# chenruduan/OAReactDiff

Measured on AMD Instinct MI355X. Metric: denoising_steps_per_sec, higher is better.
Workload: dtype f32; 1 GPU; EGNNDynamics.forward (LEFTNet H=196 R=96 L=6), B=64 reactions/GPU x 3 objects x 23 atoms, complete graph per reaction (N=4416, E=300288), T=1000 sampler step shape; batch_per_gpu=64, atoms_per_object=23, parallelism=replica x1 (no collective), launch=eager

## Files before the change

### oareactdiff_amd/_capi.py

```python
from __future__ import annotations

import ctypes as C
import os

from .build import LIB

OARD_MAX_OBJECTS = 8
ABI_VERSION = 2040
OARD_OK, OARD_EINVAL, OARD_ENOTCOMPLETE, OARD_EHIP, OARD_ENOMEM = 0, -1, -2, -3, -4
ERRORS = {OARD_EINVAL: "invalid argument / unsupported configuration", OARD_ENOTCOMPLETE: "topology is not complete-per-sample",
          OARD_EHIP: "HIP runtime error", OARD_ENOMEM: "workspace too small"}

PREC_GCL_BF16X3, PREC_EQUI_BF16X3, PREC_TRAIN_BF16X3 = 1, 2, 4
TAP_S, TAP_VEC, TAP_EDGE, TAP_POS_FRAME, TAP_DPOS, TAP_HOUT, TAP_LABELS, TAP_NE1 = 1, 2, 3, 4, 5, 6, 7, 8

EXPORTS = ["oard_version", "oard_supported", "oard_param_count", "oard_packed_bytes", "oard_pack_weights",
           "oard_topology_create", "oard_topology_destroy", "oard_topology_num_nodes", "oard_topology_num_edges",
           "oard_topology_num_inner_edges", "oard_topology_num_samples", "oard_topology_check_edge_index",
           "oard_workspace_bytes", "oard_forward", "oard_active_inner_edges", "oard_debug_lin3u_table", "oard_sampler_step", "oard_sampler_step_dev", "oard_tap", "oard_debug_stop_after", "oard_debug_option", "oard_timing_enable", "oard_timing_reset",
           "oard_timing_get",
           "oard_topology_create_parts", "oard_topology_export", "oard_tape_bytes", "oard_tape_entry", "oard_forward_train",
           "oard_packed_bwd_bytes", "oard_pack_weights_bwd", "oard_gcl_backward_dx", "oard_edge_node_sums",
           "oard_equi_backward_dx", "oard_scalarize_backward", "oard_equi_msg_backward", "oard_lin3u_forward", "oard_lin3u_backward", "oard_wgrad_scratch_bytes", "oard_wgrad",
           "oard_train_scratch_bytes", "oard_train_scratch_poison", "oard_train_scratch_entry", "oard_train_tail_backward",
# ... 99 lines not shown
    L.oard_train_stage_backward.restype = ci
    L.oard_nan_replace.argtypes = [cfgp, vp, vp, pvp, pvp, vp]; L.oard_nan_replace.restype = ci
    pf, cf = C.POINTER(C.c_float), C.c_float
    L.oard_loss_prepare.argtypes = [cfgp, vp, pvp, pvp, pvp, pvp, vp, vp, ci, pf, pf, ci, ci, pvp, pvp, vp]; L.oard_loss_prepare.restype = ci
    L.oard_loss_terms.argtypes = [cfgp, vp, pvp, pvp, pvp, pvp, pvp, vp, vp, ci, pf, pf, pf, ci, ci, vp, vp, pvp, vp]; L.oard_loss_terms.restype = ci
    cd = C.c_double
    L.oard_adamw_step.argtypes = [vp, vp, vp, vp, vp, i64, cd, cd, cd, cd, cd, i64, ci, cd, vp]; L.oard_adamw_step.restype = ci
    L.oard_adamw_step_dev.argtypes = [vp, vp, vp, vp, vp, i64, cd, cd, cd, cd, cd, ci, ci, vp, ci, vp, vp, vp, vp]; L.oard_adamw_step_dev.restype = ci
    L.oard_library_stream.argtypes = [ci, pvp]; L.oard_library_stream.restype = ci
    L.oard_graph_create.argtypes = [cfgp, vp, vp, i64, vp, i64, pvp]; L.oard_graph_create.restype = ci
    L.oard_graph_destroy.argtypes = [vp]; L.oard_graph_destroy.restype = None
    L.oard_graph_num_nodes.argtypes = [vp]; L.oard_graph_num_nodes.restype = i64
    L.oard_graph_num_edges.argtypes = [vp]; L.oard_graph_num_edges.restype = i64
    L.oard_graph_object_rows.argtypes = [vp, ci]; L.oard_graph_object_rows.restype = i64
    L.oard_graph_is_complete.argtypes = [vp]; L.oard_graph_is_complete.restype = ci
    L.oard_graph_workspace_bytes.argtypes = [cfgp, vp]; L.oard_graph_workspace_bytes.restype = sz
    L.oard_graph_forward.argtypes = [cfgp, vp, pvp, sz, pvp, vp, ci, vp, pvp, vp, sz, vp, vp]; L.oard_graph_forward.restype = ci
    L.oard_debug_stop_after.argtypes = [C.c_int]; L.oard_debug_stop_after.restype = C.c_int
    L.oard_debug_option.argtypes = [C.c_char_p, C.c_int]; L.oard_debug_option.restype = C.c_int
    L.oard_timing_enable.argtypes = [C.c_int]; L.oard_timing_enable.restype = C.c_int
    L.oard_timing_reset.argtypes = []; L.oard_timing_reset.restype = C.c_int
    L.oard_timing_get.argtypes = [C.c_char_p, C.POINTER(C.c_double), C.POINTER(i64)]; L.oard_timing_get.restype = C.c_int
    for env, opt in (("OARD_GCL_VARIANT", b"gcl_variant"), ("OARD_EQUI_VARIANT", b"equi_variant"),
                     ("OARD_NODE_VARIANT", b"node_variant"), ("OARD_GCL_SKIP", b"gcl_skip"), ("OARD_EQUI_SKIP", b"equi_skip"), ("OARD_GCL_PERSIST", b"gcl_persist"), ("OARD_GCL_GRID", b"gcl_grid"), ("OARD_PARTS", b"parts"), ("OARD_SEQUENTIAL", b"sequential"), ("OARD_POISON", b"poison"), ("OARD_AUTO_SMALL", b"auto_small"), ("OARD_AUTO_TINY", b"auto_tiny"), ("OARD_NPB", b"npb"),
                     ("OARD_WGRAD_WGS", b"wgrad_wgs"), ("OARD_WGRAD_LDS", b"wgrad_lds"), ("OARD_WGRAD_T16", b"wgrad_t16"), ("OARD_WGRAD_QUEUE", b"wgrad_queue"), ("OARD_GATE_FOLD", b"gate_fold"), ("OARD_WGRAD_SHAPES", b"wgrad_shapes"), ("OARD_TRAIN_DUAL", b"train_dual"), ("OARD_SMALL_SPLIT", b"small_split"),
                     ("OARD_SKIP_FAMILIES", b"skip_families")):
        if os.environ.get(env) not in (None, ""):
            check(L.oard_debug_option(opt, int(os.environ[env])), f"oard_debug_option({opt.decode()})")
    _lib = L
    return L


def timing_get(family: str):
    ms, n = C.c_double(0.0), C.c_int64(0)
    check(lib().oard_timing_get(family.encode(), C.byref(ms), C.byref(n)), "oard_timing_get")
    return ms.value, n.value
```

### oareactdiff_amd/csrc/oard_edge_v1.h

```cpp
#pragma once
#include "oard_kernels.h"

typedef __attribute__((address_space(3))) void* lds_ptr_t;
typedef const __attribute__((address_space(1))) void* gbl_ptr_t;

OARD_DEV void glds16(const float* gsrc_lane, float* lds_chunk);
OARD_DEV void glds16u(const float* chunk_uniform, unsigned lane_byte_off, float* lds_chunk) {
    glds16(reinterpret_cast<const float*>(reinterpret_cast<const char*>(chunk_uniform) + lane_byte_off), lds_chunk);
}
OARD_DEV void glds16(const float* gsrc_lane, float* lds_chunk) {
#ifndef OARD_ABL_NODMA_INSTR
    __builtin_amdgcn_global_load_lds((gbl_ptr_t)gsrc_lane, (lds_ptr_t)lds_chunk, 16, 0, 0);
#else
    asm volatile("" :: "v"(gsrc_lane), "s"(lds_chunk));
#endif
}

OARD_DEV void phase_barrier() {
    asm volatile("s_waitcnt vmcnt(0)" ::: "memory");
#ifndef OARD_ABL_NOBARRIER
    __syncthreads();
#endif
}

// ... 427 lines not shown
            if (TRAIN) st_f4(tape.z3 + e * D::WP + 4 * g + 16 * t, pendz[gg]);
        }
    }
    PROBE_END(pf);
    TL_END();
}

template <class D>
struct EquiStream {
    static constexpr int WB = D::WB, D1T = D::D1T, RB = D::RB, HT = D::HT;
    static constexpr int G1 = D1T, G2 = 1 + D1T + RB, NG2 = 3 * HT;
    static constexpr bool ROWS4 = (D::H % 16) >= 1 && (D::H % 16) <= 4;
    static constexpr int SLAB = G2 > G1 ? G2 : G1;
    static constexpr int NPH = WB + NG2;
    static constexpr int C1 = WB * G1, CHUNKS = C1 + NG2 * G2;
    static constexpr size_t LDS_BYTES = (size_t)2 * SLAB * 1024;
};

template <class D, int WAVES, bool TRAIN>
__global__ __launch_bounds__(WAVES * 64) void k_equi_edge_v1(TopoDev tp, const float* __restrict__ stream,
                                                             const float* __restrict__ dp0b,
                                                             const float* __restrict__ ew, const float* __restrict__ rbuf,
                                                             float* __restrict__ qbuf, float* __restrict__ zd1,
                                                             float* __restrict__ cdbuf, ActList al) {
    extern __shared__ __attribute__((aligned(16))) float smem[];
    using S = EquiStream<D>;
    constexpr int WB = D::WB, D1T = D::D1T, RB = D::RB, HT = D::HT, G1 = S::G1, G2 = S::G2;
    const int lane = threadIdx.x & 63, g = lane >> 4;
    const int wave = __builtin_amdgcn_readfirstlane(threadIdx.x >> 6);

    SlabPrefetch<WAVES, S::SLAB, 0, 3> pf;
    pf.wave = wave;
    pf.lane_off = (unsigned)lane * 16u;
    auto pf_begin = [&](int p) {
        const int start = p < WB ? p * G1 : S::C1 + (p - WB) * G2;
        pf.begin(stream, smem, p, start, p >= S::NPH ? 0 : (p < WB ? G1 : G2));
    };
    auto hook = [&]() { pf.tick(); };
    auto A = [&](int p, int j) -> f4 {
        return *reinterpret_cast<const f4*>(smem + ((size_t)(p & 1) * S::SLAB + j) * 256 + lane * 4);
    };
    auto SL = [&](int p) -> const float* { return smem + (size_t)(p & 1) * S::SLAB * 256 + lane * 4; };

    const long long n_cols = al.n != nullptr ? (long long)*al.n : tp.A;
    if ((long long)blockIdx.x * WAVES * 16 >= n_cols) return;
    const long long c = ((long long)blockIdx.x * WAVES + wave) * 16 + (lane & 15);
    const bool live = c < n_cols;
    const size_t a = (size_t)(live ? (al.rows != nullptr ? (long long)al.rows[c] : c) : tp.A);
    const float* erow = ew + (live ? a : (size_t)tp.E) * D::WP + 4 * g;
    f4 d1[D1T];
#pragma unroll
    for (int t = 0; t < D1T; ++t) d1[t] = ld_vec(dp0b, t, lane);
    f4 rb[RB];
#pragma unroll
    for (int b = 0; b < RB; ++b) rb[b] = ld_blk(rbuf, a, D::RP, b, lane);
    f4 xn = ld_f4(erow);
    pf_begin(0);
    pf.flush();

    int p = 0;
    for (int b = 0; b < WB; ++b, ++p) {
        phase_barrier();
        const f4 x = xn;
        pf_begin(p + 1);
        if (b + 1 < WB) xn = ld_f4(erow + 16 * (b + 1));
        chain_kouter<D1T>(SL(p), 0, x, d1, hook);
        pf.flush();
    }
    if (TRAIN) {
#pragma unroll
        for (int t = 0; t < D1T; ++t) st_blk(zd1, a, D::D1P, t, lane, d1[t]);
    }
#pragma unroll
    for (int t = 0; t < D1T; ++t) d1[t] = silu4(d1[t]);

    float* qrow = qbuf + a * (size_t)(3 * D::HP) + 4 * g;
    float* cdrow = TRAIN ? cdbuf + a * (size_t)(3 * D::HP) + 4 * g : nullptr;
    f4 pend = f4zero(), pendc = f4zero();
    int pend_off = 0;
    auto t2_phase = [&](int i, auto rows4) {
        phase_barrier();
        if (i > 0) {
            st_f4(qrow + pend_off, pend);
            if (TRAIN) st_f4(cdrow + pend_off, pendc);
        }
        pf_begin(p + 1);
        const int tt = i / 3, th = i - 3 * tt;
        f4 cd, cr;
        if (decltype(rows4)::value) {
            cd = reduce_g(chain_tile4<D1T>(SL(p), 1, d1, A(p, 0), hook));
            cr = reduce_g(chain_tile4<RB>(SL(p), 1 + D1T, rb, f4zero(), hook));
            if (g != 0) { cd = f4zero(); cr = f4zero(); }
        } else {
            cd = chain_tile<D1T>(SL(p), 1, d1, A(p, 0), hook);
            cr = chain_tile<RB>(SL(p), 1 + D1T, rb, f4zero(), hook);
        }
        pf.flush();
        pend = cd * cr;
        if (TRAIN) pendc = cd;
        pend_off = th * D::HP + 16 * tt;
        ++p;
    };
    constexpr int N_FULL = S::ROWS4 ? S::NG2 - 3 : S::NG2;
    for (int i = 0; i < N_FULL; ++i) t2_phase(i, std::false_type{});
    for (int i = N_FULL; i < S::NG2; ++i) t2_phase(i, std::true_type{});
    st_f4(qrow + pend_off, pend);
    if (TRAIN) st_f4(cdrow + pend_off, pendc);
}

template <class D>
__global__ __launch_bounds__(256) void k_equi_agg_v1(TopoDev tp, const float* __restrict__ wb, LayerOff lo,
                                                     const float* __restrict__ qbuf, const float* __restrict__ xq,
                                                     const float* __restrict__ geo, const float* __restrict__ x1,
                                                     float* __restrict__ s, const float* __restrict__ vec_in,
                                                     float* __restrict__ vec_out, float* __restrict__ v2buf,
                                                     float* __restrict__ scal, float* __restrict__ vdot) {
    bool live; const ColId id = col_id(tp.N, live);
    if (!live) return;
    const int n = id.col, a0 = tp.act_ptr[n], cnt = tp.act_ptr[n + 1] - a0;
    const int mx = wave_max(cnt);
    const float inv_sqrt2 = 0.70710678118654752f, inv_sqrt3 = 0.57735026918962576f,
                inv_sqrt_h = 1.0f / sqrtf((float)D::H);
    f4 vx[3][D::HT], dx[D::HT];
#pragma unroll
    for (int t = 0; t < D::HT; ++t) { dx[t] = f4zero(); vx[0][t] = f4zero(); vx[1][t] = f4zero(); vx[2][t] = f4zero(); }
    for (int k = 0; k < mx; ++k)
        if (k < cnt) {
            const size_t a = (size_t)a0 + k;
// ... 63 lines not shown
```

### oareactdiff_amd/csrc/oard_hip.hip

```cpp
#include <algorithm>
#include <cmath>
#include <cstdio>
#include <cstring>
#include <map>
#include <string>
#include <vector>
#include <mutex>
#include <chrono>
#include <utility>

#include "oard_kernels.h"
#include "oard_edge_v1.h"
#include "oard_edge_p.h"
#include "oard_wgrad_t16.h"
#include "oard_edge_b3.h"
#ifdef OARD_EXPERIMENTS
#include "oard_edge_fp.h"
#endif
#include "oard_node_v1.h"
#include "oard_edge_small.h"
#include "oard_edge_bwd.h"
#include "oard_node_bwd.h"
#include "oard_rows.h"
#include "oard_inst.h"
// ... 22 lines not shown
    hipEvent_t get() {
        if (!pool.empty()) { hipEvent_t e = pool.back(); pool.pop_back(); return e; }
        hipEvent_t e; (void)hipEventCreate(&e); return e;
    }
    void flush() {
        for (auto& r : recs) {
            (void)hipEventSynchronize(r.b);
            float ms = 0.f;
            (void)hipEventElapsedTime(&ms, r.a, r.b);
            total_ms[r.fam] += ms; launches[r.fam] += 1;
            pool.push_back(r.a); pool.push_back(r.b);
        }
        recs.clear();
    }
} g_timing;
int g_stop_after = 0;
int g_gcl_variant = 2;
int g_equi_variant = 2;
int g_sequential = 0;
int g_auto_tiny = 8;
int g_auto_small = 4;
int g_npb = 0;
int g_poison = 0;
int g_parts = 0;
int g_small_split = 128;
int g_wgrad_shapes = 3;
int g_wgrad_t16 = 256;
int g_wgrad_lds = 256;
int g_wgrad_wgs = 512;
int g_gcl_persist = 1;
int g_gcl_grid = 0;
int g_equi_skip = 1;
int g_gcl_skip = 1;
int g_node_variant = 1;
int g_skip_families = 0;

struct ScopedLaunch {
    hipStream_t st; hipEvent_t a; int fam; bool on;
    ScopedLaunch(int f, hipStream_t s) : st(s), fam(f), on(g_timing.on) {
        if (on) { a = g_timing.get(); (void)hipEventRecord(a, st); }
    }
    ~ScopedLaunch() {
        if (on) { hipEvent_t b = g_timing.get(); (void)hipEventRecord(b, st); g_timing.recs.push_back({a, b, fam}); }
    }
};
#define LAUNCH(fam, kern, grid, block, stream, ...) do { ScopedLaunch sl_(fam, stream); if (!((g_skip_families >> (fam)) & 1)) \
// ... 315 lines not shown
        case 10: { LAUNCH_LDS(F_GCL_EDGE, (k_gcl_edge_v1<D, 12, 1, S1, S3, false, 3>), cdiv(r1 - r0, 16 * 12), 12 * 64,
                              (GclStream<D, 1>::LDS_BYTES), st, tp, stream, P, Q, u0, c0, r0, r1, ew_in, ew_out, mbuf, GclTape{}); return OARD_OK; }
        case 11: { LAUNCH_LDS(F_GCL_EDGE, (k_gcl_edge_v1<D, 12, 2, S1, S3, false, 3>), cdiv(r1 - r0, 16 * 12), 12 * 64,
                              (GclStream<D, 2>::LDS_BYTES), st, tp, stream, P, Q, u0, c0, r0, r1, ew_in, ew_out, mbuf, GclTape{}); return OARD_OK; }
        case 12: { LAUNCH_LDS(F_GCL_EDGE, (k_gcl_edge_v1<D, 4, 1, S1, S3, false, 3>), cdiv(r1 - r0, 16 * 4), 4 * 64,
                              (GclStream<D, 1>::LDS_BYTES), st, tp, stream, P, Q, u0, c0, r0, r1, ew_in, ew_out, mbuf, GclTape{}); return OARD_OK; }
#endif
        default: return OARD_EINVAL;
    }
}
template <class D>
int launch_gcl_v1(int prec, int variant, int conc, const TopoDev& tp, const float* wb, const LayerOff& lo, const float* stream, const float* P, const float* Q, const float* u0,
                  const float* c0, bool first, bool last, const float* ew_in, float* ew_out, float* mbuf, const GclTape* tape, hipStream_t st) {
    const long long A = tp.A, E = tp.E;
    int rc;
    const bool skip = g_gcl_skip || tape;
    if (!skip || (!first && !last)) return launch_gcl_v1s<D, true, true>(prec, variant, conc, tp, wb, lo, stream, P, Q, u0, c0, 0, E, ew_in, ew_out, mbuf, tape, st);
    rc = launch_gcl_v1s<D, true, true>(prec, variant, conc, tp, wb, lo, stream, P, Q, u0, c0, 0, A, ew_in, ew_out, mbuf, tape, st);
    if (rc != OARD_OK) return rc;
    if (first && last) return launch_gcl_v1s<D, false, false>(prec, variant, conc, tp, wb, lo, stream, P, Q, u0, c0, A, E, ew_in, ew_out, mbuf, tape, st);
    if (first) return launch_gcl_v1s<D, false, true>(prec, variant, conc, tp, wb, lo, stream, P, Q, u0, c0, A, E, ew_in, ew_out, mbuf, tape, st);
    return launch_gcl_v1s<D, true, false>(prec, variant, conc, tp, wb, lo, stream, P, Q, u0, c0, A, E, ew_in, ew_out, mbuf, tape, st);
}
#define EQUI_CASE(id, WV_) case id: { \
        LAUNCH_LDS(F_EQUI_EDGE, (k_equi_edge_v1<D, WV_, false>), cdiv(tp.A, 16 * WV_), WV_ * 64, (EquiStream<D>::LDS_BYTES), st, \
                   tp, stream, dp0b, ew, rbuf, qbuf, nullptr, nullptr, al); return OARD_OK; }
template <class D>
int launch_equi_v1(int prec, int variant, int conc, const TopoDev& tp, const float* wb, const LayerOff& lo, const float* stream, const float* dp0b, const float* ew,
                   const float* rbuf, float* qbuf, float* zd1, float* cd, hipStream_t st, float* d1s = nullptr, ActList al = ActList{}) {
    if (zd1 && (prec & OARD_PREC_TRAIN_BF16X3) && d1s) {
        LAUNCH_LDS(F_EQUI_EDGE, (k_equi_edge_b3<D, true>), cdiv(tp.A, 16 * 8), 8 * 64, (EquiB3Stream<D>::LDS_BYTES), st, tp, wb + lo.equi_b3,
                   dp0b, wb + lo.dp2b, ew, rbuf, qbuf, d1s, zd1, cd, ActList{});
        return OARD_OK;
    }
    if (zd1) {
        LAUNCH_LDS(F_EQUI_EDGE, (k_equi_edge_v1<D, 8, true>), cdiv(tp.A, 16 * 8), 8 * 64, (EquiStream<D>::LDS_BYTES), st,
                   tp, stream, dp0b, ew, rbuf, qbuf, zd1, cd, ActList{});
        return OARD_OK;
    }
    if (variant == 2 && cdiv(tp.A, 16) * conc <= 512LL * g_auto_small) variant = 1;
    if ((variant == 2 || variant == 1) && cdiv(tp.A, 16) * conc <= 512LL * g_auto_tiny) variant = 4;
    if (variant == 4) {
        if (t_small.a && cdiv(tp.A, 16) * conc <= g_small_split) {
            const long long tiles = cdiv(tp.A, 16);
            LAUNCH_LDS(F_EQUI_EDGE, (k_equi_small_s1<D, 8>), tiles * cdiv(D::D1T, 8), 512, (size_t)D::WB * 1024, st,
                       tp, wb, lo, ew, t_small.a);
            LAUNCH_LDS(F_EQUI_EDGE, (k_equi_small_s2<D, 8>), tiles * cdiv(3 * D::HT, 8), 512, (size_t)(D::D1T + D::RB) * 1024, st,
                       tp, wb, lo, (const float*)t_small.a, rbuf, qbuf);
            return OARD_OK;
        }
        LAUNCH_LDS(F_EQUI_EDGE, (k_equi_edge_small<D, 8>), cdiv(tp.A, 16), 512, (EquiSmall<D>::LDS_BYTES), st,
                   tp, wb, lo, ew, rbuf, qbuf);
        return OARD_OK;
    }
    if (variant == 2 && (prec & OARD_PREC_EQUI_BF16X3) && d1s) {
        LAUNCH_LDS(F_EQUI_EDGE, (k_equi_edge_b3<D>), cdiv(tp.A, 16 * 8), 8 * 64, (EquiB3Stream<D>::LDS_BYTES), st, tp, wb + lo.equi_b3,
                   dp0b, wb + lo.dp2b, ew, rbuf, qbuf, d1s, nullptr, nullptr, al);
        return OARD_OK;
    }
    switch (variant) {
        EQUI_CASE(1, 4)
        EQUI_CASE(2, 8)
        default: return OARD_EINVAL;
    }
}

struct TapeOff {
    size_t hin, geo, rbuf, pp0, x1;
    size_t s_in[OARD_MAX_LAYERS + 1], vec_in[OARD_MAX_LAYERS + 1];
    size_t agg[OARD_MAX_LAYERS], s_mid[OARD_MAX_LAYERS];
    size_t s_a[OARD_MAX_LAYERS], vec_a[OARD_MAX_LAYERS];
    size_t ew[OARD_MAX_LAYERS + 1];
    size_t z1[OARD_MAX_LAYERS], z2[OARD_MAX_LAYERS], att[OARD_MAX_LAYERS], z3[OARD_MAX_LAYERS];
    size_t zd1[OARD_MAX_LAYERS], cd[OARD_MAX_LAYERS];
    size_t total;
};
static TapeOff make_tape(const oard_config* c, const TopoDev& td) {
    const RDims d(c->hidden, c->num_radial);
    const size_t N = td.N, E = td.E + 1, A = td.A + 1;
    TapeOff t;
    memset(&t, 0, sizeof(t));
    size_t cur = 0;
    auto take = [&](size_t bytes) { size_t o = cur; cur = align_up(cur + bytes, 256); return o; };
    t.hin = take(N * 16 * 4); t.geo = take(A * GEO_STRIDE * 4); t.rbuf = take(A * d.RP * 4); t.pp0 = take(N * 4); t.x1 = take(N * 3 * 4);
    for (int l = 0; l <= c->num_layers; ++l) {
// ... 101 lines not shown
                GclTape gt{};
                if (train) gt = GclTape{(float*)(tape + to.z1[l]), (float*)(tape + to.z2[l]), (float*)(tape + to.att[l]), (float*)(tape + to.z3[l])};
                int rc = launch_gcl_v1<D>(c->precision, gcl_variant, topo->conc, tp, wb, lo, wb + lo.gcl_stream, P, Q, wb + po.u0, wb + po.c0row, l == 0,
                                          l == c->num_layers - 1, ew_in, ew_out, mbuf, train ? &gt : nullptr, st);
                if (rc != OARD_OK) return rc;
            }
        }
        const bool rows = tp.npb <= 4;
        if (nv1 && rows) LAUNCH(F_NODE, (k_gcl_node_v1<D, NW, true>), gN16, NW * 64, st, tp, wb, lo, (const float*)xhb, (const float*)mbuf, s_mid_at(l), xq,
                                train ? (float*)(tape + to.agg[l]) : nullptr);
        else if (nv1) LAUNCH(F_NODE, (k_gcl_node_v1<D, NW, false>), gN16, NW * 64, st, tp, wb, lo, (const float*)xhb, (const float*)mbuf, s_mid_at(l), xq,
                             train ? (float*)(tape + to.agg[l]) : nullptr);
        else if constexpr (kV0) LAUNCH(F_NODE, (k_gcl_node<D>), gN, 256, st, tp, wb, lo, (const float*)xhb, (const float*)mbuf, s, xq);
        else return OARD_EINVAL;
        if (stop_after == 100 + 10 * l + 1) { topo->vec_final = (size_t)((char*)vcur - ws); return OARD_OK; }
        if (equi_variant == 0) {
            if constexpr (kV0) {
                if (A > 0) LAUNCH(F_EQUI_EDGE, (k_equi_edge<D>), gA, 256, st, tp, wb, lo, (const float*)ew_out, (const float*)rbuf,
                                  (const float*)geo, (const float*)xq, (const float*)vcur, xmsg, vmsg);
                LAUNCH(F_NODE, (k_equi_agg<D>), gN, 256, st, tp, wb, lo, (const float*)xmsg, (const float*)vmsg, (const float*)x1,
                       s, vcur, v2buf, scal, vdot);
            } else return OARD_EINVAL;
        } else {
            if (A > 0) {
                int rc = launch_equi_v1<D>(c->precision, equi_variant, topo->conc, tp, wb, lo, wb + lo.equi_stream, wb + lo.dp0b, ew_out, rbuf, vmsg,
                                           train ? (float*)(tape + to.zd1[l]) : nullptr, train ? (float*)(tape + to.cd[l]) : nullptr, st,
                                           (float*)(ws + w.d1s), al);
                if (rc != OARD_OK) return rc;
            }
#define EQUI_NODE_V1(ROWS_, XC_) LAUNCH(F_NODE, (k_equi_node_v1<D, NW, ROWS_, XC_>), gN16, NW * 64, st, tp, wb, lo, (const float*)vmsg, \
                       (const float*)xq, (const float*)geo, (const float*)x1, (const float*)s_mid_at(l), s_at(l + 1), (const float*)vcur, vnext, \
                       train ? (float*)(tape + to.s_a[l]) : nullptr, train ? (float*)(tape + to.vec_a[l]) : nullptr, al)
            if (nv1 && rows) {
                if (lo.xcross) EQUI_NODE_V1(true, true); else EQUI_NODE_V1(true, false);
            } else if (nv1) {
                if (lo.xcross) EQUI_NODE_V1(false, true); else EQUI_NODE_V1(false, false);
            } else if constexpr (kV0) {
                LAUNCH(F_NODE, (k_equi_agg_v1<D>), gN, 256, st, tp, wb, lo, (const float*)vmsg, (const float*)xq,
                       (const float*)geo, (const float*)x1, s, (const float*)vcur, vnext, v2buf, scal, vdot);
            } else return OARD_EINVAL;
            std::swap(vcur, vnext);
        }
        if constexpr (kV0) {
            if (!nv1) LAUNCH(F_NODE, (k_equi_upd<D>), gN, 256, st, tp, wb, lo, (const float*)scal, (const float*)vdot,
                             (const float*)v2buf, s, vcur);
        }
        if (stop_after == 100 + 10 * l + 2) { topo->vec_final = (size_t)((char*)vcur - ws); return OARD_OK; }
    }
    if (!train) topo->vec_final = (size_t)((char*)vcur - ws);
    if (train) {
        ZeroRows z;
        z.count = 0;
        auto add = [&](size_t off, size_t row, int ld) {
            if (z.count == 64) { LAUNCH(F_OTHER, k_zero_rows, 64, 256, st, z); z.count = 0; }
            z.p[z.count] = (float*)(tape + off) + row * (size_t)ld; z.n[z.count] = ld; ++z.count;
        };
        for (int l = 0; l <= c->num_layers; ++l) {
            add(to.ew[l], (size_t)E, D::WP);
            if (l == c->num_layers) break;
// ... 1478 lines not shown
            case OARD_TAP_EDGE:
                if (tp.E > 0)
                    hipLaunchKernelGGL(k_tap_edges, dim3((unsigned)cdiv(tp.E * d.W, 256)), dim3(256), 0, st, tp,
                                       (const float*)(ws + w.ew), d.WP, d.W, dst);
                break;
            default: return OARD_EINVAL;
        }
    }
    HIP_TRY(hipGetLastError());
    return OARD_OK;
}

int oard_debug_stop_after(int code) { g_stop_after = code; return OARD_OK; }
int oard_debug_option(const char* name, int value) {
    if (!name) return OARD_EINVAL;
    if (!kV0 && value == 0 && (strcmp(name, "gcl_variant") == 0 || strcmp(name, "equi_variant") == 0 || strcmp(name, "node_variant") == 0))
        return OARD_EINVAL;
    if (strcmp(name, "gcl_variant") == 0) { g_gcl_variant = value; return OARD_OK; }
    if (strcmp(name, "equi_variant") == 0) { g_equi_variant = value; return OARD_OK; }
    if (strcmp(name, "node_variant") == 0) { g_node_variant = value; return OARD_OK; }
    if (strcmp(name, "experiments") == 0) return kV0 ? OARD_OK : OARD_EINVAL;
    if (strcmp(name, "gcl_skip") == 0) { g_gcl_skip = value; return OARD_OK; }
    if (strcmp(name, "equi_skip") == 0) { g_equi_skip = value; return OARD_OK; }
    if (strcmp(name, "gcl_persist") == 0) { g_gcl_persist = value; return OARD_OK; }
    if (strcmp(name, "gcl_grid") == 0) { g_gcl_grid = value; return OARD_OK; }
    if (strcmp(name, "skip_families") == 0) { g_skip_families = value; return OARD_OK; }
    if (strcmp(name, "parts") == 0) { g_parts = value; return OARD_OK; }
    if (strcmp(name, "sequential") == 0) { g_sequential = value; return OARD_OK; }
    if (strcmp(name, "poison") == 0) { g_poison = value; return OARD_OK; }
    if (strcmp(name, "auto_small") == 0) { g_auto_small = value; return OARD_OK; }
    if (strcmp(name, "auto_tiny") == 0) { g_auto_tiny = value; return OARD_OK; }
    if (strcmp(name, "npb") == 0) { g_npb = value; return OARD_OK; }
    if (strcmp(name, "wgrad_wgs") == 0) { g_wgrad_wgs = value; return OARD_OK; }
    if (strcmp(name, "wgrad_t16") == 0) { g_wgrad_t16 = value; return OARD_OK; }
    if (strcmp(name, "wgrad_queue") == 0) { g_wgrad_queue = value; return OARD_OK; }
    if (strcmp(name, "gate_fold") == 0) { g_gate_fold = value; return OARD_OK; }
    if (strcmp(name, "wgrad_lds") == 0) { g_wgrad_lds = value; return OARD_OK; }
    if (strcmp(name, "wgrad_shapes") == 0) { g_wgrad_shapes = value & 3; return OARD_OK; }
    if (strcmp(name, "train_dual") == 0) { g_train_dual = value; return OARD_OK; }
    if (strcmp(name, "small_split") == 0) { g_small_split = value; return OARD_OK; }
    return OARD_EINVAL;
}
#ifdef OARD_PHASE_PROBE
int oard_debug_probe_read(unsigned long long* out8) {
    if (!out8) return OARD_EINVAL;
    HIP_TRY(hipDeviceSynchronize());
// ... 38 lines not shown
```

### oareactdiff_amd/csrc/oard_inst.h

```cpp
#pragma once
#if !defined(OARD_EXPERIMENTS) && !defined(OARD_SINGLE_TU)

#define OARD_UNPAREN(...) __VA_ARGS__
#ifdef OARD_INST_DEFINE
#define OARD_INST(K, ARGS) template __global__ void OARD_UNPAREN K ARGS;
#else
#define OARD_INST(K, ARGS) extern template __global__ void OARD_UNPAREN K ARGS;
#endif
#ifndef OARD_DIMS_LIST
#define OARD_DIMS_LIST X(196, 96) X(32, 8) X(32, 32)
#endif
#define OARD_BOOL4(M, D) M(D, true, true) M(D, false, true) M(D, true, false) M(D, false, false)

#define OARD_NW(h) (((h) + 15) / 16 <= 16 ? ((h) + 15) / 16 : 8)
#define OARD_A_GCL (TopoDev, const float*, const float*, const float*, const float*, const float*, long long, long long, const float*, float*, float*, GclTape)

#if !defined(OARD_INST_DEFINE) || defined(OARD_INST_UNIT_GCL_P)
#define OARD_I_GCL_P(D, S1, S3) OARD_INST((k_gcl_edge_p<OARD_UNPAREN D, S1, S3, false>), OARD_A_GCL) OARD_INST((k_gcl_edge_p<OARD_UNPAREN D, S1, S3, true>), OARD_A_GCL)
#define X(h, r) OARD_BOOL4(OARD_I_GCL_P, (Dims<h, r>))
OARD_DIMS_LIST
#undef X
#endif

#if !defined(OARD_INST_DEFINE) || defined(OARD_INST_UNIT_GCL_V1)
#define OARD_I_GCL_V1(D, S1, S3) \
    OARD_INST((k_gcl_edge_v1<OARD_UNPAREN D, 8, 2, S1, S3, false, 2, 3>), OARD_A_GCL) OARD_INST((k_gcl_edge_v1<OARD_UNPAREN D, 8, 2, S1, S3, true, 2, 3>), OARD_A_GCL) \
    OARD_INST((k_gcl_edge_v1<OARD_UNPAREN D, 4, 2, S1, S3, false, 2, 2>), OARD_A_GCL) \
    OARD_INST((k_gcl_edge_small<OARD_UNPAREN D, 8, S1, S3>), (TopoDev, const float*, LayerOff, const float*, const float*, const float*, const float*, long long, long long, float*, float*))
#define X(h, r) OARD_BOOL4(OARD_I_GCL_V1, (Dims<h, r>))
OARD_DIMS_LIST
#undef X
#endif

#if !defined(OARD_INST_DEFINE) || defined(OARD_INST_UNIT_B3)
#define OARD_A_EQUI_B3 (TopoDev, const float*, const float*, const float*, const float*, const float*, float*, float*, float*, float*, ActList)
#define OARD_I_GCL_B3(D, S1, S3) OARD_INST((k_gcl_edge_b3<OARD_UNPAREN D, S1, S3, false>), OARD_A_GCL) OARD_INST((k_gcl_edge_b3<OARD_UNPAREN D, S1, S3, true>), OARD_A_GCL)
#define X(h, r) OARD_BOOL4(OARD_I_GCL_B3, (Dims<h, r>)) OARD_INST((k_equi_edge_b3<Dims<h, r>, false>), OARD_A_EQUI_B3) OARD_INST((k_equi_edge_b3<Dims<h, r>, true>), OARD_A_EQUI_B3)
OARD_DIMS_LIST
#undef X
#endif

#if !defined(OARD_INST_DEFINE) || defined(OARD_INST_UNIT_EQUI)
#define OARD_A_EQUI (TopoDev, const float*, const float*, const float*, const float*, float*, float*, float*, ActList)
#define OARD_A_EQUI_NODE (TopoDev, const float*, LayerOff, const float*, const float*, const float*, const float*, const float*, float*, const float*, float*, float*, float*, ActList)
#define X(h, r) \
    OARD_INST((k_equi_edge_v1<Dims<h, r>, 8, false>), OARD_A_EQUI) OARD_INST((k_equi_edge_v1<Dims<h, r>, 8, true>), OARD_A_EQUI) \
    OARD_INST((k_equi_edge_v1<Dims<h, r>, 4, false>), OARD_A_EQUI) \
    OARD_INST((k_equi_node_v1<Dims<h, r>, OARD_NW(h), false, false>), OARD_A_EQUI_NODE) OARD_INST((k_equi_node_v1<Dims<h, r>, OARD_NW(h), false, true>), OARD_A_EQUI_NODE) \
    OARD_INST((k_equi_node_v1<Dims<h, r>, OARD_NW(h), true, false>), OARD_A_EQUI_NODE) OARD_INST((k_equi_node_v1<Dims<h, r>, OARD_NW(h), true, true>), OARD_A_EQUI_NODE) \
    OARD_INST((k_gcl_edge_bwd<Dims<h, r>, 8, 2, true>), (TopoDev, const float*, long long, long long, GclBwdArgs)) \
    OARD_INST((k_gcl_edge_bwd<Dims<h, r>, 8, 2, false>), (TopoDev, const float*, long long, long long, GclBwdArgs)) \
    OARD_INST((k_equi_edge_bwd<Dims<h, r>, 8>), (TopoDev, const float*, const float*, const float*, float*, float*))
OARD_DIMS_LIST
#undef X
#endif

#if !defined(OARD_INST_DEFINE) || defined(OARD_INST_UNIT_NODE)
#define OARD_A_GCL_NODE (TopoDev, const float*, LayerOff, const float*, const float*, float*, float*, float*)
#define OARD_A_OUT (TopoDev, const float*, PackOff, const float*, const float*, float*, float*, int*)
#define OARD_A_SCAL_BWD (TopoDev, const float*, const float*, int, const float*, const float*, float*, float*)
#define OARD_A_MSG_BWD (TopoDev, const float*, Strided3, Strided3, const float*, Strided3, const float*, int, Strided3, float*, float*, float*, float*, int, int, int)
#define X(h, r) \
    OARD_INST((k_gcl_node_v1<Dims<h, r>, OARD_NW(h), false>), OARD_A_GCL_NODE) OARD_INST((k_gcl_node_v1<Dims<h, r>, OARD_NW(h), true>), OARD_A_GCL_NODE) \
    OARD_INST((k_out_v1<Dims<h, r>, OARD_NW(h)>), OARD_A_OUT) \
    OARD_INST((k_scalarize_bwd<Dims<h, r>, 2, false>), OARD_A_SCAL_BWD) OARD_INST((k_scalarize_bwd<Dims<h, r>, 2, true>), OARD_A_SCAL_BWD) \
    OARD_INST((k_equi_msg_bwd<Dims<h, r> >), OARD_A_MSG_BWD)
OARD_DIMS_LIST
#undef X
OARD_INST((k_lin3u_bwd_fused<4>), (const float*, const float*, const float*, long long, float*, float*))
#define OARD_I_ROWS(KB, EPI) OARD_INST((k_rows_dense<KB, EPI, 8>), (RowsDense)) OARD_INST((k_rows_dense_long<KB, EPI, 8, 4>), (RowsDense))
OARD_I_ROWS(13, 0) OARD_I_ROWS(13, 2) OARD_I_ROWS(13, 3) OARD_I_ROWS(7, 3) OARD_I_ROWS(6, 0) OARD_I_ROWS(6, 1) OARD_I_ROWS(4, 1) OARD_I_ROWS(4, 3)
OARD_INST((k_rows_dense<26, 1, 8>), (RowsDense)) OARD_INST((k_rows_dense<26, 3, 8>), (RowsDense))
// ... 16 lines not shown
```

### oareactdiff_amd/csrc/oard_node_v1.h

```cpp
#pragma once
#include "oard_kernels.h"

OARD_DEV f4 lds_blk(const float* v, int b, int lane) { return *reinterpret_cast<const f4*>(v + b * 256 + lane * 4); }
OARD_DEV void lds_st(float* v, int t, int lane, f4 x) { *reinterpret_cast<f4*>(v + t * 256 + lane * 4) = x; }

#ifndef OARD_NODE_PF
#define OARD_NODE_PF 13
#endif
template <int KB>
OARD_DEV f4 dense_tile_lds(const float* __restrict__ wp, int t, const float* in, int lane, f4 init) {
    const float* base = wp + ((size_t)t * KB * 64 + lane) * 4;
    f4 c0 = init, c1 = f4zero();
    constexpr int G = OARD_NODE_PF;
#pragma unroll
    for (int b0 = 0; b0 < KB; b0 += G) {
        f4 a[G];
#pragma unroll
        for (int i = 0; i < G; ++i)
            if (b0 + i < KB) a[i] = ld_f4(base + (size_t)(b0 + i) * 256);
        __builtin_amdgcn_sched_barrier(0);
#pragma unroll
        for (int i = 0; i < G; ++i)
            if (b0 + i < KB) {
                const f4 x = lds_blk(in, b0 + i, lane);
// ... 399 lines not shown
    for (int j = 0; j < 8; ++j) o += silu4(h2[j]) * w4[j];
    return o;
}

OARD_DEV float lin3u1(const float* l3s, const float* __restrict__ p, float x) {
    const float* b2 = p + 576;
    const float* w4 = p + 584;
    float h2[8];
#pragma unroll
    for (int j = 0; j < 8; ++j) h2[j] = b2[j];
#pragma unroll 4
    for (int k = 0; k < 48; ++k) {
        const f4 wa = *reinterpret_cast<const f4*>(l3s + 12 * k), wc = *reinterpret_cast<const f4*>(l3s + 12 * k + 4);
        const float h = silu1(x * l3s[12 * k + 8] + l3s[12 * k + 9]);
        h2[0] += h * wa.x; h2[1] += h * wa.y; h2[2] += h * wa.z; h2[3] += h * wa.w;
        h2[4] += h * wc.x; h2[5] += h * wc.y; h2[6] += h * wc.z; h2[7] += h * wc.w;
    }
    float o = p[592];
#pragma unroll
    for (int j = 0; j < 8; ++j) o += silu1(h2[j]) * w4[j];
    return o;
}

template <class D, int WAVES, bool ROWS = false, bool XC = false>
__global__ __launch_bounds__(WAVES * 64) void k_equi_node_v1(TopoDev tp, const float* __restrict__ wb, LayerOff lo,
                                                             const float* __restrict__ qbuf, const float* __restrict__ xq,
                                                             const float* __restrict__ geo, const float* __restrict__ x1,
                                                             const float* s, float* s_out, const float* __restrict__ vec_in,
                                                             float* __restrict__ vec_out,
                                                             float* __restrict__ sa_out, float* __restrict__ va_out ,
                                                             ActList al ) {
    constexpr int HT = D::HT;
    constexpr int TPW = (HT + WAVES - 1) / WAVES;
    __shared__ __attribute__((aligned(16))) float sm[6 * HT * 256 + 48 * 12 + L3T_FLOATS];
    float* l3s = sm + 6 * HT * 256;
    float* l3t = l3s + 48 * 12;
#ifdef OARD_NO_L3T
    const bool l3t_ok = false;
#else
    const bool l3t_ok = tp.npb > 4 && (wb + lo.l3t)[2 * (L3T_N + 1)] > 0.5f;
#endif
    if (l3t_ok)
        for (int i = threadIdx.x; i < 2 * (L3T_N + 1) / 4; i += WAVES * 64)
            reinterpret_cast<f4*>(l3t)[i] = ld_f4(wb + lo.l3t + 4 * i);
    if (l3t_ok && threadIdx.x < 2) l3t[2 * (L3T_N + 1) - 2 + threadIdx.x] = (wb + lo.l3t)[2 * (L3T_N + 1) - 2 + threadIdx.x];
#ifdef OARD_TIMELINE
    const bool tl_on_ = blockIdx.x == gridDim.x / 2 && (threadIdx.x & 63) == 0; int tl_n_ = 0;
#endif
    TL(1);
    lin3u_stage(wb + lo.l3u, l3s, threadIdx.x, WAVES * 64);
    float* vx = sm;
    float* in = sm + 3 * HT * 256;
    float* hx = sm + 5 * HT * 256;
    const NodeBlk nb = node_blk(tp.N, tp.npb);
// ... 35 lines not shown
                const f4 w0 = ld_blk(vec_in, (size_t)m * 3 + 0, D::HP, t, nb.lane), w1 = ld_blk(vec_in, (size_t)m * 3 + 1, D::HP, t, nb.lane),
                         w2 = ld_blk(vec_in, (size_t)m * 3 + 2, D::HP, t, nb.lane);
                if (kk < cnt2) {
                    const f4 xm = (y0 + zn0) * q0;
                    dx += xm;
                    const f4 a2 = (y1 + zn1) * q1 * inv_sqrt3;
                    const f4 a3 = (y2 + zn2) * q2;
                    v0 += (XC ? w0 * a2 + a3 * gx + xm * cx : w0 * a2 + a3 * gx) * inv_sqrt_h;
                    v1 += (XC ? w1 * a2 + a3 * gy + xm * cy : w1 * a2 + a3 * gy) * inv_sqrt_h;
                    v2 += (XC ? w2 * a2 + a3 * gz + xm * cz : w2 * a2 + a3 * gz) * inv_sqrt_h;
                }
            }
            dx = rows_total4(dx, rl, nb.lane); v0 = rows_total4(v0, rl, nb.lane);
            v1 = rows_total4(v1, rl, nb.lane); v2 = rows_total4(v2, rl, nb.lane);
        }
        int mnext[2], rnext[2];
        auto entry = [&](int kk, int& m, int& r) {
            const int ke = min(a0 + min(kk, max(cnt - 1, 0)), a_hi);
            m = cnt > 0 ? src_of(ke) : 0;
            r = cnt > 0 ? row_of(ke) : 0;
        };
#pragma unroll
        for (int i = 0; i < 2; ++i) entry(i, mnext[i], rnext[i]);
        for (int k = 0; !ROWS && k < mx; k += 2) {
            f4 q0[2], q1[2], q2[2], y0[2], y1[2], y2[2], w0[2], w1[2], w2[2];
            float gx[2], gy[2], gz[2], cx[2], cy[2], cz[2];
            const int mc[2] = {mnext[0], mnext[1]}, rc[2] = {rnext[0], rnext[1]};
#pragma unroll
            for (int i = 0; i < 2; ++i)
                entry(k + 2 + i, mnext[i], rnext[i]);
#pragma unroll
            for (int i = 0; i < 2; ++i) {
                const size_t a = (size_t)rc[i];
                const int m = mc[i];
                const float* g = geo + a * GEO_STRIDE;
                gx[i] = g[2]; gy[i] = g[3]; gz[i] = g[4];
                cx[i] = XC ? g[5] : 0.f; cy[i] = XC ? g[6] : 0.f; cz[i] = XC ? g[7] : 0.f;
                q0[i] = ld_blk(qbuf, a, 3 * D::HP, t, nb.lane); q1[i] = ld_blk(qbuf, a, 3 * D::HP, HT + t, nb.lane);
                q2[i] = ld_blk(qbuf, a, 3 * D::HP, 2 * HT + t, nb.lane);
                y0[i] = ld_blk(xq, m, 3 * D::HP, t, nb.lane); y1[i] = ld_blk(xq, m, 3 * D::HP, HT + t, nb.lane);
                y2[i] = ld_blk(xq, m, 3 * D::HP, 2 * HT + t, nb.lane);
                w0[i] = ld_blk(vec_in, (size_t)m * 3 + 0, D::HP, t, nb.lane);
                w1[i] = ld_blk(vec_in, (size_t)m * 3 + 1, D::HP, t, nb.lane);
                w2[i] = ld_blk(vec_in, (size_t)m * 3 + 2, D::HP, t, nb.lane);
            }
#pragma unroll
            for (int i = 0; i < 2; ++i)
                if (k + i < cnt) {
                    const f4 xm = (y0[i] + xn0) * q0[i];
                    dx += xm;
                    const f4 a2 = (y1[i] + xn1) * q1[i] * inv_sqrt3;
                    const f4 a3 = (y2[i] + xn2) * q2[i];
                    v0 += (XC ? w0[i] * a2 + a3 * gx[i] + xm * cx[i] : w0[i] * a2 + a3 * gx[i]) * inv_sqrt_h;
                    v1 += (XC ? w1[i] * a2 + a3 * gy[i] + xm * cy[i] : w1[i] * a2 + a3 * gy[i]) * inv_sqrt_h;
                    v2 += (XC ? w2[i] * a2 + a3 * gz[i] + xm * cz[i] : w2[i] * a2 + a3 * gz[i]) * inv_sqrt_h;
                }
        }
        const f4 sa = (ld_blk(s, n, D::HP, t, nb.lane) + dx) * inv_sqrt2;
        v0 += ld_blk(vec_in, (size_t)n * 3 + 0, D::HP, t, nb.lane);
        v1 += ld_blk(vec_in, (size_t)n * 3 + 1, D::HP, t, nb.lane);
        v2 += ld_blk(vec_in, (size_t)n * 3 + 2, D::HP, t, nb.lane);
        lds_st(in, t, nb.lane, sa);
        lds_st(vx + 0 * HT * 256, t, nb.lane, v0);
        lds_st(vx + 1 * HT * 256, t, nb.lane, v1);
        lds_st(vx + 2 * HT * 256, t, nb.lane, v2);
        if (sa_out != nullptr && nb.valid) {
            st_blk(sa_out, n, D::HP, t, nb.lane, sa);
// ... 316 lines not shown
```

Before: 3597 reaction-steps/s.

## Skip the middle equivariant message third at layer 0 where input vectors are zero

At layer 0 the incoming vector features are zero, so the middle channel group of the equivariant edge message (the term multiplied by vec_in) contributes nothing. The edge kernel gains a skip flag that steps over every third G2 prefetch/compute slot, and a Layer0 specialization of the node kernel stops loading q1, y1 and vec_in, substituting an opaque zero. This removes edge GEMM work, stores and gathers for that layer. It assumes vec_in really is zero at layer 0 and is restricted to inference with variant 2.

Result: faster. 3638 reaction-steps/s, median of 6 (+1.1%).

```diff
diff --git a/oareactdiff_amd/_capi.py b/oareactdiff_amd/_capi.py
--- a/oareactdiff_amd/_capi.py
+++ b/oareactdiff_amd/_capi.py
@@ -145,7 +145,7 @@
     L.oard_timing_reset.argtypes = []; L.oard_timing_reset.restype = C.c_int
     L.oard_timing_get.argtypes = [C.c_char_p, C.POINTER(C.c_double), C.POINTER(i64)]; L.oard_timing_get.restype = C.c_int
     for env, opt in (("OARD_GCL_VARIANT", b"gcl_variant"), ("OARD_EQUI_VARIANT", b"equi_variant"),
-                     ("OARD_NODE_VARIANT", b"node_variant"), ("OARD_GCL_SKIP", b"gcl_skip"), ("OARD_EQUI_SKIP", b"equi_skip"), ("OARD_GCL_PERSIST", b"gcl_persist"), ("OARD_GCL_GRID", b"gcl_grid"), ("OARD_PARTS", b"parts"), ("OARD_SEQUENTIAL", b"sequential"), ("OARD_POISON", b"poison"), ("OARD_AUTO_SMALL", b"auto_small"), ("OARD_AUTO_TINY", b"auto_tiny"), ("OARD_NPB", b"npb"),
+                     ("OARD_NODE_VARIANT", b"node_variant"), ("OARD_GCL_SKIP", b"gcl_skip"), ("OARD_EQUI_SKIP", b"equi_skip"), ("OARD_EQUI_L0_SKIP", b"equi_l0_skip"), ("OARD_GCL_PERSIST", b"gcl_persist"), ("OARD_GCL_GRID", b"gcl_grid"), ("OARD_PARTS", b"parts"), ("OARD_SEQUENTIAL", b"sequential"), ("OARD_POISON", b"poison"), ("OARD_AUTO_SMALL", b"auto_small"), ("OARD_AUTO_TINY", b"auto_tiny"), ("OARD_NPB", b"npb"),
                      ("OARD_WGRAD_WGS", b"wgrad_wgs"), ("OARD_WGRAD_LDS", b"wgrad_lds"), ("OARD_WGRAD_T16", b"wgrad_t16"), ("OARD_WGRAD_QUEUE", b"wgrad_queue"), ("OARD_GATE_FOLD", b"gate_fold"), ("OARD_WGRAD_SHAPES", b"wgrad_shapes"), ("OARD_TRAIN_DUAL", b"train_dual"), ("OARD_SMALL_SPLIT", b"small_split"),
                      ("OARD_SKIP_FAMILIES", b"skip_families")):
         if os.environ.get(env) not in (None, ""):
diff --git a/oareactdiff_amd/csrc/oard_edge_v1.h b/oareactdiff_amd/csrc/oard_edge_v1.h
--- a/oareactdiff_amd/csrc/oard_edge_v1.h
+++ b/oareactdiff_amd/csrc/oard_edge_v1.h
@@ -473,7 +473,7 @@
                                                              const float* __restrict__ dp0b,
                                                              const float* __restrict__ ew, const float* __restrict__ rbuf,
                                                              float* __restrict__ qbuf, float* __restrict__ zd1,
-                                                             float* __restrict__ cdbuf, ActList al) {
+                                                             float* __restrict__ cdbuf, ActList al, int skip_mid) {
     extern __shared__ __attribute__((aligned(16))) float smem[];
     using S = EquiStream<D>;
     constexpr int WB = D::WB, D1T = D::D1T, RB = D::RB, HT = D::HT, G1 = S::G1, G2 = S::G2;
@@ -483,10 +483,14 @@
     SlabPrefetch<WAVES, S::SLAB, 0, 3> pf;
     pf.wave = wave;
     pf.lane_off = (unsigned)lane * 16u;
-    auto pf_begin = [&](int p) {
-        const int start = p < WB ? p * G1 : S::C1 + (p - WB) * G2;
-        pf.begin(stream, smem, p, start, p >= S::NPH ? 0 : (p < WB ? G1 : G2));
-    };
+    const bool skip = !TRAIN && skip_mid != 0;
+    auto pf_begin = [&](int ph) {
+        pf.begin(stream, smem, ph, ph * G1, G1);
+    };
+    auto pf_begin_t2 = [&](int ph, int slot) {
+        pf.begin(stream, smem, ph, S::C1 + slot * G2, slot < S::NG2 ? G2 : 0);
+    };
+    auto next_slot = [&](int i) -> int { return i + ((skip && i % 3 == 0) ? 2 : 1); };
     auto hook = [&]() { pf.tick(); };
     auto A = [&](int p, int j) -> f4 {
         return *reinterpret_cast<const f4*>(smem + ((size_t)(p & 1) * S::SLAB + j) * 256 + lane * 4);
@@ -513,7 +517,7 @@
     for (int b = 0; b < WB; ++b, ++p) {
         phase_barrier();
         const f4 x = xn;
-        pf_begin(p + 1);
+        if (b + 1 < WB) pf_begin(p + 1); else pf_begin_t2(p + 1, 0);
         if (b + 1 < WB) xn = ld_f4(erow + 16 * (b + 1));
         chain_kouter<D1T>(SL(p), 0, x, d1, hook);
         pf.flush();
@@ -535,7 +539,7 @@
             st_f4(qrow + pend_off, pend);
             if (TRAIN) st_f4(cdrow + pend_off, pendc);
         }
-        pf_begin(p + 1);
+        pf_begin_t2(p + 1, next_slot(i));
         const int tt = i / 3, th = i - 3 * tt;
         f4 cd, cr;
         if (decltype(rows4)::value) {
@@ -553,8 +557,8 @@
         ++p;
     };
     constexpr int N_FULL = S::ROWS4 ? S::NG2 - 3 : S::NG2;
-    for (int i = 0; i < N_FULL; ++i) t2_phase(i, std::false_type{});
-    for (int i = N_FULL; i < S::NG2; ++i) t2_phase(i, std::true_type{});
+    for (int i = 0; i < N_FULL; i = next_slot(i)) t2_phase(i, std::false_type{});
+    for (int i = N_FULL; i < S::NG2; i = next_slot(i)) t2_phase(i, std::true_type{});
     st_f4(qrow + pend_off, pend);
     if (TRAIN) st_f4(cdrow + pend_off, pendc);
 }
diff --git a/oareactdiff_amd/csrc/oard_hip.hip b/oareactdiff_amd/csrc/oard_hip.hip
--- a/oareactdiff_amd/csrc/oard_hip.hip
+++ b/oareactdiff_amd/csrc/oard_hip.hip
@@ -68,6 +68,8 @@
 int g_auto_small = 4;
 int g_npb = 0;
 int g_poison = 0;
+int g_equi_l0_skip = 1;
+int g_equi_l0_taken = 0;
 int g_parts = 0;
 int g_small_split = 128;
 int g_wgrad_shapes = 3;
@@ -429,12 +431,18 @@
     if (first) return launch_gcl_v1s<D, false, true>(prec, variant, conc, tp, wb, lo, stream, P, Q, u0, c0, A, E, ew_in, ew_out, mbuf, tape, st);
     return launch_gcl_v1s<D, true, false>(prec, variant, conc, tp, wb, lo, stream, P, Q, u0, c0, A, E, ew_in, ew_out, mbuf, tape, st);
 }
-#define EQUI_CASE(id, WV_) case id: { \
+static int equi_v1_shape(int prec, int variant, int conc, long long A, const float* d1s) {
+    if (variant == 2 && cdiv(A, 16) * conc <= 512LL * g_auto_small) variant = 1;
+    if ((variant == 2 || variant == 1) && cdiv(A, 16) * conc <= 512LL * g_auto_tiny) variant = 4;
+    if (variant == 2 && (prec & OARD_PREC_EQUI_BF16X3) && d1s) variant = 5;
+    return variant;
+}
+#define EQUI_CASE(id, WV_, SKIP_) case id: { \
         LAUNCH_LDS(F_EQUI_EDGE, (k_equi_edge_v1<D, WV_, false>), cdiv(tp.A, 16 * WV_), WV_ * 64, (EquiStream<D>::LDS_BYTES), st, \
-                   tp, stream, dp0b, ew, rbuf, qbuf, nullptr, nullptr, al); return OARD_OK; }
+                   tp, stream, dp0b, ew, rbuf, qbuf, nullptr, nullptr, al, SKIP_); return OARD_OK; }
 template <class D>
 int launch_equi_v1(int prec, int variant, int conc, const TopoDev& tp, const float* wb, const LayerOff& lo, const float* stream, const float* dp0b, const float* ew,
-                   const float* rbuf, float* qbuf, float* zd1, float* cd, hipStream_t st, float* d1s = nullptr, ActList al = ActList{}) {
+                   const float* rbuf, float* qbuf, float* zd1, float* cd, hipStream_t st, float* d1s = nullptr, ActList al = ActList{}, bool skip_mid = false) {
     if (zd1 && (prec & OARD_PREC_TRAIN_BF16X3) && d1s) {
         LAUNCH_LDS(F_EQUI_EDGE, (k_equi_edge_b3<D, true>), cdiv(tp.A, 16 * 8), 8 * 64, (EquiB3Stream<D>::LDS_BYTES), st, tp, wb + lo.equi_b3,
                    dp0b, wb + lo.dp2b, ew, rbuf, qbuf, d1s, zd1, cd, ActList{});
@@ -442,11 +450,11 @@
     }
     if (zd1) {
         LAUNCH_LDS(F_EQUI_EDGE, (k_equi_edge_v1<D, 8, true>), cdiv(tp.A, 16 * 8), 8 * 64, (EquiStream<D>::LDS_BYTES), st,
-                   tp, stream, dp0b, ew, rbuf, qbuf, zd1, cd, ActList{});
+                   tp, stream, dp0b, ew, rbuf, qbuf, zd1, cd, ActList{}, 0);
         return OARD_OK;
     }
-    if (variant == 2 && cdiv(tp.A, 16) * conc <= 512LL * g_auto_small) variant = 1;
-    if ((variant == 2 || variant == 1) && cdiv(tp.A, 16) * conc <= 512LL * g_auto_tiny) variant = 4;
+    variant = equi_v1_shape(prec, variant, conc, tp.A, d1s);
+    if (skip_mid && variant != 2) return OARD_EINVAL;
     if (variant == 4) {
         if (t_small.a && cdiv(tp.A, 16) * conc <= g_small_split) {
             const long long tiles = cdiv(tp.A, 16);
@@ -460,14 +468,14 @@
                    tp, wb, lo, ew, rbuf, qbuf);
         return OARD_OK;
     }
-    if (variant == 2 && (prec & OARD_PREC_EQUI_BF16X3) && d1s) {
+    if (variant == 5) {
         LAUNCH_LDS(F_EQUI_EDGE, (k_equi_edge_b3<D>), cdiv(tp.A, 16 * 8), 8 * 64, (EquiB3Stream<D>::LDS_BYTES), st, tp, wb + lo.equi_b3,
                    dp0b, wb + lo.dp2b, ew, rbuf, qbuf, d1s, nullptr, nullptr, al);
         return OARD_OK;
     }
     switch (variant) {
-        EQUI_CASE(1, 4)
-        EQUI_CASE(2, 8)
+        EQUI_CASE(1, 4, 0)
+        EQUI_CASE(2, 8, skip_mid ? 1 : 0)
         default: return OARD_EINVAL;
     }
 }
@@ -615,19 +623,24 @@
                        s, vcur, v2buf, scal, vdot);
             } else return OARD_EINVAL;
         } else {
+            const bool l0_skip = l == 0 && !train && g_equi_l0_skip && A > 0 && nv1 && !rows &&
+                                 equi_v1_shape(c->precision, equi_variant, topo->conc, A, (const float*)(ws + w.d1s)) == 2;
+            if (l == 0) g_equi_l0_taken = l0_skip;
             if (A > 0) {
                 int rc = launch_equi_v1<D>(c->precision, equi_variant, topo->conc, tp, wb, lo, wb + lo.equi_stream, wb + lo.dp0b, ew_out, rbuf, vmsg,
                                            train ? (float*)(tape + to.zd1[l]) : nullptr, train ? (float*)(tape + to.cd[l]) : nullptr, st,
-                                           (float*)(ws + w.d1s), al);
+                                           (float*)(ws + w.d1s), al, l0_skip);
                 if (rc != OARD_OK) return rc;
             }
-#define EQUI_NODE_V1(ROWS_, XC_) LAUNCH(F_NODE, (k_equi_node_v1<D, NW, ROWS_, XC_>), gN16, NW * 64, st, tp, wb, lo, (const float*)vmsg, \
+#define EQUI_NODE_V1(D_, ROWS_, XC_) LAUNCH(F_NODE, (k_equi_node_v1<D_, NW, ROWS_, XC_>), gN16, NW * 64, st, tp, wb, lo, (const float*)vmsg, \
                        (const float*)xq, (const float*)geo, (const float*)x1, (const float*)s_mid_at(l), s_at(l + 1), (const float*)vcur, vnext, \
                        train ? (float*)(tape + to.s_a[l]) : nullptr, train ? (float*)(tape + to.vec_a[l]) : nullptr, al)
             if (nv1 && rows) {
-                if (lo.xcross) EQUI_NODE_V1(true, true); else EQUI_NODE_V1(true, false);
+                if (lo.xcross) EQUI_NODE_V1(D, true, true); else EQUI_NODE_V1(D, true, false);
+            } else if (nv1 && l0_skip) {
+                if (lo.xcross) EQUI_NODE_V1(Layer0<D>, false, true); else EQUI_NODE_V1(Layer0<D>, false, false);
             } else if (nv1) {
-                if (lo.xcross) EQUI_NODE_V1(false, true); else EQUI_NODE_V1(false, false);
+                if (lo.xcross) EQUI_NODE_V1(D, false, true); else EQUI_NODE_V1(D, false, false);
             } else if constexpr (kV0) {
                 LAUNCH(F_NODE, (k_equi_agg_v1<D>), gN, 256, st, tp, wb, lo, (const float*)vmsg, (const float*)xq,
                        (const float*)geo, (const float*)x1, s, (const float*)vcur, vnext, v2buf, scal, vdot);
@@ -2152,6 +2165,8 @@
     if (strcmp(name, "experiments") == 0) return kV0 ? OARD_OK : OARD_EINVAL;
     if (strcmp(name, "gcl_skip") == 0) { g_gcl_skip = value; return OARD_OK; }
     if (strcmp(name, "equi_skip") == 0) { g_equi_skip = value; return OARD_OK; }
+    if (strcmp(name, "equi_l0_skip") == 0) { g_equi_l0_skip = value; return OARD_OK; }
+    if (strcmp(name, "equi_l0_taken") == 0) return g_equi_l0_taken ? OARD_OK : OARD_EINVAL;
     if (strcmp(name, "gcl_persist") == 0) { g_gcl_persist = value; return OARD_OK; }
     if (strcmp(name, "gcl_grid") == 0) { g_gcl_grid = value; return OARD_OK; }
     if (strcmp(name, "skip_families") == 0) { g_skip_families = value; return OARD_OK; }
diff --git a/oareactdiff_amd/csrc/oard_inst.h b/oareactdiff_amd/csrc/oard_inst.h
--- a/oareactdiff_amd/csrc/oard_inst.h
+++ b/oareactdiff_amd/csrc/oard_inst.h
@@ -41,13 +41,14 @@
 #endif
 
 #if !defined(OARD_INST_DEFINE) || defined(OARD_INST_UNIT_EQUI)
-#define OARD_A_EQUI (TopoDev, const float*, const float*, const float*, const float*, float*, float*, float*, ActList)
+#define OARD_A_EQUI (TopoDev, const float*, const float*, const float*, const float*, float*, float*, float*, ActList, int)
 #define OARD_A_EQUI_NODE (TopoDev, const float*, LayerOff, const float*, const float*, const float*, const float*, const float*, float*, const float*, float*, float*, float*, ActList)
 #define X(h, r) \
     OARD_INST((k_equi_edge_v1<Dims<h, r>, 8, false>), OARD_A_EQUI) OARD_INST((k_equi_edge_v1<Dims<h, r>, 8, true>), OARD_A_EQUI) \
     OARD_INST((k_equi_edge_v1<Dims<h, r>, 4, false>), OARD_A_EQUI) \
     OARD_INST((k_equi_node_v1<Dims<h, r>, OARD_NW(h), false, false>), OARD_A_EQUI_NODE) OARD_INST((k_equi_node_v1<Dims<h, r>, OARD_NW(h), false, true>), OARD_A_EQUI_NODE) \
     OARD_INST((k_equi_node_v1<Dims<h, r>, OARD_NW(h), true, false>), OARD_A_EQUI_NODE) OARD_INST((k_equi_node_v1<Dims<h, r>, OARD_NW(h), true, true>), OARD_A_EQUI_NODE) \
+    OARD_INST((k_equi_node_v1<Layer0<Dims<h, r> >, OARD_NW(h), false, false>), OARD_A_EQUI_NODE) OARD_INST((k_equi_node_v1<Layer0<Dims<h, r> >, OARD_NW(h), false, true>), OARD_A_EQUI_NODE) \
     OARD_INST((k_gcl_edge_bwd<Dims<h, r>, 8, 2, true>), (TopoDev, const float*, long long, long long, GclBwdArgs)) \
     OARD_INST((k_gcl_edge_bwd<Dims<h, r>, 8, 2, false>), (TopoDev, const float*, long long, long long, GclBwdArgs)) \
     OARD_INST((k_equi_edge_bwd<Dims<h, r>, 8>), (TopoDev, const float*, const float*, const float*, float*, float*))
diff --git a/oareactdiff_amd/csrc/oard_node_v1.h b/oareactdiff_amd/csrc/oard_node_v1.h
--- a/oareactdiff_amd/csrc/oard_node_v1.h
+++ b/oareactdiff_amd/csrc/oard_node_v1.h
@@ -445,6 +445,9 @@
     return o;
 }
 
+template <class D> struct Layer0 : D {};
+template <class D> struct is_layer0 { static constexpr bool value = false; };
+template <class D> struct is_layer0<Layer0<D> > { static constexpr bool value = true; };
 template <class D, int WAVES, bool ROWS = false, bool XC = false>
 __global__ __launch_bounds__(WAVES * 64) void k_equi_node_v1(TopoDev tp, const float* __restrict__ wb, LayerOff lo,
                                                              const float* __restrict__ qbuf, const float* __restrict__ xq,
@@ -453,6 +456,8 @@
                                                              float* __restrict__ vec_out,
                                                              float* __restrict__ sa_out, float* __restrict__ va_out ,
                                                              ActList al ) {
+    constexpr bool L0 = is_layer0<D>::value;
+    static_assert(!(L0 && ROWS), "the layer-0 form exists for the large-batch gather only");
     constexpr int HT = D::HT;
     constexpr int TPW = (HT + WAVES - 1) / WAVES;
     __shared__ __attribute__((aligned(16))) float sm[6 * HT * 256 + 48 * 12 + L3T_FLOATS];
@@ -534,6 +539,9 @@
         };
 #pragma unroll
         for (int i = 0; i < 2; ++i) entry(i, mnext[i], rnext[i]);
+        float zero1 = 0.f;
+        if (L0) asm volatile("" : "+v"(zero1));
+        const f4 zero4 = {zero1, zero1, zero1, zero1};
         for (int k = 0; !ROWS && k < mx; k += 2) {
             f4 q0[2], q1[2], q2[2], y0[2], y1[2], y2[2], w0[2], w1[2], w2[2];
             float gx[2], gy[2], gz[2], cx[2], cy[2], cz[2];
@@ -548,13 +556,13 @@
                 const float* g = geo + a * GEO_STRIDE;
                 gx[i] = g[2]; gy[i] = g[3]; gz[i] = g[4];
                 cx[i] = XC ? g[5] : 0.f; cy[i] = XC ? g[6] : 0.f; cz[i] = XC ? g[7] : 0.f;
-                q0[i] = ld_blk(qbuf, a, 3 * D::HP, t, nb.lane); q1[i] = ld_blk(qbuf, a, 3 * D::HP, HT + t, nb.lane);
+                q0[i] = ld_blk(qbuf, a, 3 * D::HP, t, nb.lane); q1[i] = L0 ? zero4 : ld_blk(qbuf, a, 3 * D::HP, HT + t, nb.lane);
                 q2[i] = ld_blk(qbuf, a, 3 * D::HP, 2 * HT + t, nb.lane);
-                y0[i] = ld_blk(xq, m, 3 * D::HP, t, nb.lane); y1[i] = ld_blk(xq, m, 3 * D::HP, HT + t, nb.lane);
+                y0[i] = ld_blk(xq, m, 3 * D::HP, t, nb.lane); y1[i] = L0 ? zero4 : ld_blk(xq, m, 3 * D::HP, HT + t, nb.lane);
                 y2[i] = ld_blk(xq, m, 3 * D::HP, 2 * HT + t, nb.lane);
-                w0[i] = ld_blk(vec_in, (size_t)m * 3 + 0, D::HP, t, nb.lane);
-                w1[i] = ld_blk(vec_in, (size_t)m * 3 + 1, D::HP, t, nb.lane);
-                w2[i] = ld_blk(vec_in, (size_t)m * 3 + 2, D::HP, t, nb.lane);
+                w0[i] = L0 ? zero4 : ld_blk(vec_in, (size_t)m * 3 + 0, D::HP, t, nb.lane);
+                w1[i] = L0 ? zero4 : ld_blk(vec_in, (size_t)m * 3 + 1, D::HP, t, nb.lane);
+                w2[i] = L0 ? zero4 : ld_blk(vec_in, (size_t)m * 3 + 2, D::HP, t, nb.lane);
             }
 #pragma unroll
             for (int i = 0; i < 2; ++i)
```
